# apache/brpc

Hardware: NVIDIA H100
Metric: echo QPS, 1 KB baidu_std (higher is better)
Workload: dtype u8

## Files before the change

brpc_b200/csrc/b2_api.cu:

```cuda
#include <cuda_runtime.h>
#include <dlfcn.h>
#include <stdio.h>
#include <time.h>
#include <stdlib.h>
#include <string.h>
#include <algorithm>
#include <mutex>
#include <string>
#include <unordered_map>
#include <vector>
#include "b2_kernels.cuh"
#include "b2_h2.cuh"

using namespace b2;

static thread_local char g_err[512] = "";
static void set_err(const char* fmt, const char* a = "", const char* b = "") { snprintf(g_err, sizeof g_err, fmt, a, b); }

#define CU(call)                                                                          \
    do {                                                                                  \
        cudaError_t e_ = (call);                                                          \
        if (e_ != cudaSuccess) { set_err("%s: %s", #call, cudaGetErrorString(e_)); return B2_E_CUDA; } \
    } while (0)

// ... 21 lines not shown
    ulonglong2* d_iov = nullptr; b2_iovec* h_iov = nullptr; const void* host_bytes = nullptr;
    uint4* d_refs = nullptr; b2_resp_ref* h_refs = nullptr; int input_mode = B2_INPUT_COPY, resp_mode = B2_RESP_COPY; const uint8_t* pull_bytes = nullptr; uint32_t small_off_refs = 0;
    uint32_t* d_crc_adv = nullptr; unsigned long long* d_counters = nullptr; uint32_t* d_totals = nullptr; DevMethod* d_methods = nullptr;
    size_t meta_tile_off = 0; uint32_t max_tiles = 0; uint32_t n_sms = 132; bool use_tma_pack = true; uint32_t stage_mask = 7;
    StreamPass sp = {}; bool has_streams = false, stream_armed = false, stream_ran = false, stream_valid = false;
    uint32_t st_max = 0, st_open = 0; std::vector<long long> st_keys; std::vector<uint8_t> st_state; std::vector<uint32_t> st_pool, st_pool_free;
    void* d_st_block[10] = {}; void* h_st_mapped[5] = {}; uint32_t* h_st_cnts = nullptr; uint8_t* h_st_out = nullptr; uint8_t* h_st_ctl = nullptr; uint8_t* d_st_ctl = nullptr;
    b2_stream_msg* h_st_msgs = nullptr; b2_stream_event* h_st_events = nullptr; uint8_t* h_st_ctrl = nullptr; uint32_t* h_st_run_ctrl = nullptr;
    cudaEvent_t st_ev[6] = {};
    const uint8_t* st_input = nullptr;
    void* d_sw[4] = {}; size_t sw_have[4] = {}; SwRec* h_sw_recs = nullptr; size_t h_sw_have = 0; uint32_t* h_sw_cnts = nullptr;
    cudaEvent_t sw_ev[8] = {}; bool sw_ran = false;
    b2_run_status* h_run_status = nullptr; b2_msg_desc* h_msgs = nullptr; uint8_t* h_resp = nullptr;
    uint32_t* h_totals = nullptr; uint32_t* h_run_tile_base = nullptr;
    uint32_t n_runs = 0, n_tiles = 0, nbytes = 0, max_run_tiles = 0; uint64_t covered = 0;
    bool uploaded = false, executed = false;
    cudaStream_t stream = nullptr;
    cudaEvent_t ev[kMaxStages + 1];
    const char* stage_names[kMaxStages];
    int n_stages = 0;
    float last_kernel_ms = 0.f; uint32_t last_launches = 0;
    cudaEvent_t ev_first = nullptr, ev_last = nullptr; bool first_pending = true;
    bool profile_stages = false; bool allow_small = true; bool use_fused = true; bool fused_last = false; bool slow_heavy = false;
    bool adaptive_tile = false; bool dense = false; uint32_t avg_frame = 0;
    uint8_t* d_meta = nullptr; uint8_t* h_meta = nullptr;
    uint8_t* d_small = nullptr; uint8_t* h_small = nullptr;
    bool small = false, small_copy_queued = false, use_fused_small = true; uint32_t small_msgs = 0, small_resp = 0, small_off_rs = 0, small_off_msgs = 0, small_off_resp = 0, small_total = 0;
};

static void input_overwritten(b2_ctx* c) { if (c->st_input == c->d_bytes) c->st_input = nullptr; }

static uint32_t g_crc_tab_host[256];
static void crc_table_init() {
    for (uint32_t i = 0; i < 256; i++) {
        uint32_t c = i;
        for (int k = 0; k < 8; k++) c = (c & 1) ? (c >> 1) ^ 0x82f63b78u : (c >> 1);
        g_crc_tab_host[i] = c;
    }
}

extern "C" const char* b2_last_error(void) { return g_err; }
extern "C" const char* b2_version(void) { return "brpc_b200 0.1 (sm_90a)"; }

namespace {
struct BlockPool {
    std::mutex mu;
    static constexpr size_t kSmall = 8192, kSlab = 4u << 20;
// ... 136 lines not shown
    CU(cudaStreamCreateWithFlags(&c->stream, cudaStreamNonBlocking));
    for (int i = 0; i <= kMaxStages; i++) CU(cudaEventCreate(&c->ev[i]));
    CU(cudaEventCreate(&c->ev_first)); CU(cudaEventCreate(&c->ev_last));
    crc_table_init();
    CU(cudaMemcpyToSymbol(c_crc_table, g_crc_tab_host, sizeof g_crc_tab_host));
    {
        std::vector<uint32_t> tab(kCrcHotWords + kCrcTreeWords);
        auto adv = [&](uint32_t x, int bytes) { for (int k = 0; k < bytes; k++) x = g_crc_tab_host[x & 0xff] ^ (x >> 8); return x; };
        for (int k = 0; k < 16; k++) for (uint32_t b = 0; b < 256; b++) tab[k * 256 + b] = adv(g_crc_tab_host[b], k);
        for (int j = 0; j < 4; j++) for (uint32_t b = 0; b < 256; b++) tab[(16 + j) * 256 + b] = adv(b << (8 * j), 512);
        for (int t = 0; t < 5; t++) for (int j = 0; j < 4; j++) for (uint32_t b = 0; b < 256; b++)
            tab[kCrcHotWords + (t * 4 + j) * 256 + b] = adv(b << (8 * j), 16 << t);
        CU(cudaMemcpy(c->d_crc_adv, tab.data(), tab.size() * 4, cudaMemcpyHostToDevice));
    }
    CU(cudaFuncSetAttribute(k_resolve, cudaFuncAttributeMaxDynamicSharedMemorySize, 200 * 1024));
    CU(cudaFuncSetAttribute(k_pack_slow<false>, cudaFuncAttributeMaxDynamicSharedMemorySize, (int)(8 * kSnapRing)));
    CU(cudaFuncSetAttribute(k_pack_tma<kPackGroup>, cudaFuncAttributeMaxDynamicSharedMemorySize, (int)(sizeof(PackWarpSmem) * kPackWarps)));
    CU(cudaFuncSetAttribute(k_pack_tma<kPackGroupSmall>, cudaFuncAttributeMaxDynamicSharedMemorySize, (int)(sizeof(PackWarpSmem) * kPackWarps)));
    if (const char* e = getenv("B2_PACK")) c->use_tma_pack = strcmp(e, "reg") != 0;
    if (const char* e = getenv("B2_SMALL")) c->use_fused_small = strcmp(e, "off") != 0;
    if (const char* e = getenv("B2_FUSED")) c->use_fused = strcmp(e, "off") != 0;
    CU(cudaFuncSetAttribute(k_fused, cudaFuncAttributeMaxDynamicSharedMemorySize, (int)(sizeof(FusedWarpSmem) * (kFusedWarps > kFusedWarpsDense ? kFusedWarps : kFusedWarpsDense))));
    CU(cudaFuncSetAttribute(k_small, cudaFuncAttributeMaxDynamicSharedMemorySize, (int)sizeof(SmallSmem)));
    *out = c;
    return B2_OK;
}

extern "C" int b2_set_server_identity(b2_ctx* c, const char* ip_port) {
    if (!c) return B2_E_INVAL;
    const size_t n = ip_port ? strlen(ip_port) : 0;
    if (n >= sizeof c->cfg.identity) { set_err("identity too long"); return B2_E_INVAL; }
    memset(c->cfg.identity, 0, sizeof c->cfg.identity);
    if (n) memcpy(c->cfg.identity, ip_port, n);
    c->cfg.identity_len = (uint32_t)n;
    return B2_OK;
}

extern "C" int b2_set_modes(b2_ctx* c, int input_mode, int resp_mode) {
    if (!c || (input_mode != B2_INPUT_COPY && input_mode != B2_INPUT_PULL) || (resp_mode != B2_RESP_COPY && resp_mode != B2_RESP_BY_REF && resp_mode != B2_RESP_IOVEC)) { set_err("bad mode"); return B2_E_INVAL; }
    static_assert(sizeof(b2_resp_ref) == sizeof(uint4), "b2_resp_ref is 16 bytes");
    static_assert(sizeof(b2_iovec) == sizeof(ulonglong2) && sizeof(void*) == 8, "b2_iovec is a 16-byte struct iovec");
    if (resp_mode == B2_RESP_IOVEC && !c->d_iov) {
        CU(cudaSetDevice(c->opt.device));
        if (cudaMalloc((void**)&c->d_iov, 32 * (size_t)c->opt.max_msgs) != cudaSuccess || cudaHostAlloc((void**)&c->h_iov, 32 * (size_t)c->opt.max_msgs, cudaHostAllocDefault) != cudaSuccess) {
            cudaFree(c->d_iov); c->d_iov = nullptr; cudaGetLastError(); set_err("allocation of the iovec list failed"); return B2_E_NOMEM;
        }
// ... 52 lines not shown

static BatchPtrs make_ptrs(b2_ctx* c) {
    BatchPtrs B;
    B.bytes = c->d_bytes; B.runs = c->d_runs; B.run_tile_base = c->d_run_tile_base; B.tiles = c->d_tiles;
    B.tile_base = c->d_tile_base; B.tile_scratch = c->d_tile_scratch; B.tile_spec = c->d_tile_spec; B.run_status = c->d_run_status; B.frame_off = c->d_frame_off; B.frame_run = c->d_frame_run; B.frame_row = c->d_frame_row; B.rows = c->d_rows; B.msgs = c->d_msgs;
    B.aux = c->d_aux; B.jobs = c->d_jobs; B.refs = c->d_refs; B.slow_idx = c->d_slow_idx; B.heads = c->d_heads; B.slot = c->d_slot; B.scan_tmp = c->d_scan_tmp; B.resp = c->d_resp; B.unz = c->d_unz; B.snappy_tab = c->d_snappy_tab; B.counters = c->d_counters;
    B.totals = c->d_totals; B.methods = c->d_methods; B.crc_adv = c->d_crc_adv;
    B.n_runs = c->n_runs; B.n_tiles = c->n_tiles; B.max_msgs = c->opt.max_msgs; B.max_resp = c->opt.max_resp_bytes;
    B.runs = reinterpret_cast<const b2_run*>(c->d_meta);
    B.run_tile_base = reinterpret_cast<const uint32_t*>(c->d_meta + (size_t)c->n_runs * sizeof(b2_run));
    B.tile_info = reinterpret_cast<const uint4*>(c->d_meta + c->meta_tile_off);
    if (c->input_mode == B2_INPUT_PULL) B.bytes = c->pull_bytes;
    if (c->small) {
        B.refs = reinterpret_cast<uint4*>(c->d_small + c->small_off_refs);
        B.totals = reinterpret_cast<uint32_t*>(c->d_small);
        B.run_status = reinterpret_cast<b2_run_status*>(c->d_small + c->small_off_rs);
        B.msgs = reinterpret_cast<b2_msg_desc*>(c->d_small + c->small_off_msgs);
        B.resp = c->d_small + c->small_off_resp;
        B.max_msgs = c->small_msgs; B.max_resp = c->small_resp;
    }
    return B;
}

extern "C" int b2_batch_upload(b2_ctx* c, const void* bytes, uint32_t nbytes, const b2_run* runs, uint32_t n_runs) {
    if (!c || (!bytes && nbytes) || (!runs && n_runs)) { set_err("null argument"); return B2_E_INVAL; }
    if ((c->input_mode != B2_INPUT_PULL && nbytes > c->opt.max_batch_bytes) || nbytes >= (1u << 31) || n_runs > c->opt.max_runs) { set_err("batch exceeds ctx capacity"); return B2_E_CAPACITY; }
    uint64_t covered = 0; for (uint32_t r = 0; r < n_runs; r++) covered += runs[r].length;
    if (c->input_mode == B2_INPUT_PULL && covered > c->opt.max_batch_bytes) { set_err("runs exceed ctx capacity"); return B2_E_CAPACITY; }
    c->stream_valid = false;
    c->covered = covered;
    CU(cudaSetDevice(c->opt.device));
    if (c->adaptive_tile) {
        uint32_t t = 8192;
        const uint32_t per_tile = c->input_mode == B2_INPUT_PULL ? 48u : 6u;
        if (c->input_mode == B2_INPUT_PULL && t < 32768) t = 32768;
        while (t < (1u << 20) && t < per_tile * c->avg_frame) t <<= 1;
        c->cfg.tile_bytes = t; c->cfg.tile_shift = 0; while ((1u << c->cfg.tile_shift) < t) c->cfg.tile_shift++;
    }
    const uint32_t shift = c->cfg.tile_shift, tile = c->cfg.tile_bytes;
    c->dense = tile >= 2048 && c->avg_frame && (uint64_t)c->avg_frame * kSpecK < tile;
    c->cfg.spec_k = c->dense ? kSpecKDense : kSpecK;
    uint64_t nt = 0; uint32_t max_rt = 0;
    for (uint32_t r = 0; r < n_runs; r++) {
        if ((runs[r].offset & 15u) || (uint64_t)runs[r].offset + runs[r].length > nbytes) { set_err("run offset must be 16-aligned and inside the batch"); return B2_E_INVAL; }
        c->h_run_tile_base[r] = (uint32_t)nt;
        const uint32_t t = (uint32_t)(((uint64_t)runs[r].length + tile - 1) >> shift);
        nt += t; if (t > max_rt) max_rt = t;
    }
    c->h_run_tile_base[n_runs] = (uint32_t)nt;
    if (nt > c->max_tiles) { set_err("too many tiles"); return B2_E_CAPACITY; }
    c->n_runs = n_runs; c->n_tiles = (uint32_t)nt; c->nbytes = nbytes; c->max_run_tiles = max_rt; c->host_bytes = bytes;
    const size_t tile_off = ((size_t)n_runs * sizeof(b2_run) + 4 * ((size_t)n_runs + 1) + 15) & ~(size_t)15;
    const size_t meta_bytes = tile_off + 16 * (size_t)nt;
    c->meta_tile_off = tile_off;
    if (n_runs) memcpy(c->h_meta, runs, (size_t)n_runs * sizeof(b2_run));
    memcpy(c->h_meta + (size_t)n_runs * sizeof(b2_run), c->h_run_tile_base, 4 * ((size_t)n_runs + 1));
    {
        uint32_t* ti = reinterpret_cast<uint32_t*>(c->h_meta + tile_off);
        for (uint32_t r = 0; r < n_runs; r++) {
            const uint32_t t0 = c->h_run_tile_base[r], t1 = c->h_run_tile_base[r + 1];
            for (uint32_t t = t0; t < t1; t++) { uint32_t* q = ti + 4 * (size_t)t; q[0] = runs[r].offset; q[1] = runs[r].length; q[2] = t - t0; q[3] = r | (runs[r].flags << 24); }
        }
    }
// ... 22 lines not shown

static const char* const kStreamStages[5] = { "stream_route", "stream_alloc", "stream_group", "stream_run", "stream_rst" };
static int launch_stream_pass(b2_ctx* c, const BatchPtrs& B, cudaStream_t s, uint32_t& launches) {
    const StreamPass& S = c->sp;
    const uint32_t msg_bound = c->small ? c->small_msgs : c->opt.max_msgs, sms = c->n_sms;
    auto grid = [&](uint32_t items, uint32_t per_block, uint32_t most) { const uint32_t g = (items + per_block - 1) / per_block; return g < 1 ? 1u : g < most ? g : most; };
    CU(cudaMemsetAsync(S.cnts, 0, 4 * (16 + 2 * (size_t)S.cap), s));
    CU(cudaEventRecord(c->st_ev[0], s));
    k_stream_route<<<grid(msg_bound, 256, sms * 4), 256, 0, s>>>(B, S); CU(cudaEventRecord(c->st_ev[1], s));
    k_stream_alloc<<<grid(c->st_max, 256, sms), 256, 0, s>>>(B, S); CU(cudaEventRecord(c->st_ev[2], s));
    k_stream_group<<<grid(msg_bound, 256, sms * 4), 256, 0, s>>>(B, S); CU(cudaEventRecord(c->st_ev[3], s));
    k_stream_run<<<grid(c->st_max, 4, sms * 8), 128, 0, s>>>(B, S); CU(cudaEventRecord(c->st_ev[4], s));
    k_stream_rst<<<grid(c->n_runs, 4, sms * 4), 128, 0, s>>>(B, S); CU(cudaEventRecord(c->st_ev[5], s));
    CU(cudaMemcpyAsync(c->h_st_cnts, S.cnts, 64, cudaMemcpyDeviceToHost, s));
    launches += 5; c->stream_ran = true; c->st_input = B.bytes;
    return B2_OK;
}

static int launch_pipeline(b2_ctx* c) {
    const BatchPtrs B = make_ptrs(c);
    DevConfig C = c->cfg;
    const bool fused = c->use_fused && !c->slow_heavy && !c->small && c->input_mode == B2_INPUT_COPY && c->resp_mode == B2_RESP_COPY && c->use_tma_pack &&
                       (((uint64_t)c->nbytes + 255) & ~255ull) + 4096 <= c->opt.max_resp_bytes;
    C.fused = fused ? 1u : 0u; C.ovf_base = (c->nbytes + 255u) & ~255u; c->fused_last = fused;
    cudaStream_t s = c->stream;
    int st = 0; uint32_t launches = 0;
    const bool prof = c->profile_stages;
    auto mark = [&](const char* name) { if (prof) { c->stage_names[st] = name; cudaEventRecord(c->ev[st + 1], s); st++; } };
    const uint32_t mask = c->stage_mask;
    if (mask & 1) CU(cudaMemsetAsync(B.totals, 0, 48, s));
    CU(cudaEventRecord(c->ev[0], s));
    c->stream_ran = false;
    if (c->n_runs == 0) { c->n_stages = 0; c->last_launches = 0; return B2_OK; }
    if (c->small && c->use_fused_small && !prof) {
        k_small<<<1, kSmallThreads, sizeof(SmallSmem), s>>>(B, C);
        launches = 1;
        if (c->stream_armed) { int rc = launch_stream_pass(c, B, s, launches); if (rc != B2_OK) return rc; }
        c->stage_names[0] = "fused_small"; cudaEventRecord(c->ev[1], s);
        c->n_stages = 1; c->last_launches = launches;
        CU(cudaGetLastError());
        return B2_OK;
    }
    const uint32_t sms = c->n_sms;
    if (mask & 1) {
    if (c->n_tiles) {
        k_tile_search<<<(c->n_tiles * 32 + 255) / 256, 256, 0, s>>>(B, C); launches++; mark("tile_search");
        if (C.pull) k_tile_walk_pull<<<(uint32_t)(((uint64_t)c->n_tiles * 8 + 127) / 128), 128, 0, s>>>(B, C);
        else k_tile_walk<<<(c->n_tiles + 127) / 128, 128, 0, s>>>(B, C);
        launches++; mark("tile_walk");
    }
    {
        size_t smem = (size_t)c->max_run_tiles * 12;
        if (smem > 200 * 1024) smem = 0;
        k_resolve<<<c->n_runs, 256, smem, s>>>(B, C, smem == 0 ? 1u : 0u); launches++; mark("resolve");
    }
    if (fused) {
        const uint32_t fw = c->avg_frame && !c->dense ? kFusedWarps : kFusedWarpsDense;
        if (c->n_tiles) { k_fused<<<sms, fw * 32, sizeof(FusedWarpSmem) * fw, s>>>(B, C); launches++; mark("fused"); }
    } else {
    if (c->n_tiles) { k_frame_table<<<(uint32_t)(((uint64_t)c->n_tiles * C.spec_k + 255) / 256), 256, 0, s>>>(B, C); launches++; mark("frame_table"); }
    k_decode<<<sms * B2_DECODE_MIN_BLOCKS, kDecodeWarps * 32, 0, s>>>(B, C); launches++; mark("decode");
    k_scan_blocks<<<sms, kScanBlock, 0, s>>>(B); launches++;
    mark("scan");
    }
    }
    if (fused) {
        if (mask & 4) { k_pack_slow<true><<<sms * B2_SLOW_MIN_BLOCKS, 256, 0, s>>>(B, C); launches++; mark("pack_slow"); }
    } else if (c->use_tma_pack) {
        if (mask & 4) {
            if (c->slow_heavy || c->cfg.by_ref) { C.verify_done = 1; k_crc_verify<<<sms * 6, 256, 0, s>>>(B, C); launches++; mark("crc_verify"); }
            k_pack_slow<false><<<sms * B2_SLOW_MIN_BLOCKS, 256, 8 * kSnapRing, s>>>(B, C); launches++; mark("pack_slow");
        }
        if (mask & 2) {
            if ((c->avg_frame && c->avg_frame < 640) || c->cfg.by_ref) k_pack_tma<kPackGroupSmall><<<sms, kPackWarps * 32, sizeof(PackWarpSmem) * kPackWarps, s>>>(B, C);
            else k_pack_tma<kPackGroup><<<sms, kPackWarps * 32, sizeof(PackWarpSmem) * kPackWarps, s>>>(B, C);
            launches++; mark("pack");
        }
    } else { k_pack<<<sms * B2_PACK_MIN_BLOCKS, 256, 0, s>>>(B, C); launches++; mark("pack"); }
    if (c->resp_mode == B2_RESP_IOVEC && !c->small) {
        k_emit_iov<<<sms * 4, 256, 0, s>>>(B, c->d_iov, (unsigned long long)(uintptr_t)c->h_resp, (unsigned long long)(uintptr_t)c->host_bytes);
        launches++; mark("emit_iov");
    }
    if (c->stream_armed) { int rc = launch_stream_pass(c, B, s, launches); if (rc != B2_OK) return rc; }
    if (!prof) { c->stage_names[0] = "pipeline"; cudaEventRecord(c->ev[1], s); st = 1; }
    c->n_stages = st; c->last_launches = launches;
    CU(cudaGetLastError());
    return B2_OK;
}

extern "C" int b2_batch_execute(b2_ctx* c, float* kernel_ms, uint32_t* n_launches) {
    if (!c || !c->uploaded) { set_err("no batch uploaded"); return B2_E_INVAL; }
    CU(cudaSetDevice(c->opt.device));
    if (c->stream_armed) { set_err("a submitted batch of a context with a stream table must be collected first: this entry point replays a batch and does not run the stream pass"); return B2_E_INVAL; }
    c->profile_stages = true;
    int rc = launch_pipeline(c);
    c->profile_stages = false;
    if (rc != B2_OK) return rc;
// ... 1230 lines not shown
```

brpc_b200/csrc/b2_kernels.cuh:

```cuda
#pragma once
#include <cuda_runtime.h>
#include "b2_core.cuh"
#include "b2_inflate.cuh"

namespace b2 {

enum TileKind : uint8_t { kRanOff = 0, kStop = 1, kAmbig = 2 };

struct __align__(16) TileRec {
    uint32_t entry;
    uint32_t exit;
    uint32_t count;
    uint8_t kind;
    int8_t last_proto;
    uint8_t live;
    int8_t pf_in;
};

struct __align__(16) MsgAux {
    uint32_t msg_off;
    uint32_t msg_len;
    uint32_t att_len;
    uint32_t att_off;
    uint32_t cks_off;
// ... 14 lines not shown
constexpr uint32_t kHeadBytes = 96;

enum ErrKind : uint32_t { kErrNone = 0, kErrAttachment, kErrNoService, kErrNoMethod, kErrParseRequest };

struct DevMethod {
    char full_method[200];
    uint32_t full_method_len;
    char service_short[64];  uint32_t service_short_len;
    char service_full[120];  uint32_t service_full_len;
    char request_type[96];   uint32_t request_type_len;
    int32_t handler, echo_attachment, response_checksum_type, response_compress_type;
};
struct DevConfig {
    uint64_t max_body_size;
    uint32_t tile_bytes, tile_shift;
    uint32_t n_methods;
    uint32_t identity_len;
    uint32_t stream_handler;
    uint32_t spec_k;
    uint32_t by_ref;
    uint32_t verify_done;
    uint32_t proto_mask;
    uint32_t fused;
    uint32_t ovf_base;
    uint32_t pull_vecs;
    uint32_t pull;
    char identity[64];
};

struct BatchPtrs {
    const uint8_t* bytes;
    const b2_run* runs;
    const uint32_t* run_tile_base;
    const uint4* tile_info;
    TileRec* tiles;
    uint32_t* tile_base;
    uint32_t* tile_scratch;
    uint32_t* tile_spec;
    b2_run_status* run_status;
    uint32_t* frame_off;
    uint32_t* frame_run;
    uint32_t* frame_row;
    uint4* rows;
    b2_msg_desc* msgs;
    MsgAux* aux;
    PackJob* jobs;
// ... 29 lines not shown
}
struct NoEmit { B2_HD void operator()(uint32_t, const Step&) const {} };
constexpr uint32_t kSpecK = 16;
constexpr uint32_t kSpecKDense = 128;
constexpr uint8_t kKindRewalked = 0x80;
struct EmitSpec {
    uint32_t* out; uint32_t run_off, cap;
    __device__ __forceinline__ void operator()(uint32_t i, const Step& s) const {
        if (i < cap) out[i] = (run_off + s.frame_pos) | ((uint32_t)(s.index != 1) << 31);
    }
};

#if defined(__CUDACC__)

__device__ __forceinline__ uint32_t find_run(const uint32_t* base, uint32_t n_runs, uint32_t tile) {
    uint32_t lo = 0, hi = n_runs;
    while (hi - lo > 1) { const uint32_t mid = (lo + hi) >> 1; if (__ldg(base + mid) <= tile) lo = mid; else hi = mid; }
    return lo;
}
__device__ __forceinline__ bool is_magic(uint32_t w) { return w == kMagicPRPC || w == kMagicSTRM; }
#ifndef B2_SEARCH_FIRST
#define B2_SEARCH_FIRST 2
#endif

__global__ void __launch_bounds__(256, 6) k_tile_search(BatchPtrs B, DevConfig C) {
    const uint32_t warp = (blockIdx.x * blockDim.x + threadIdx.x) >> 5, lane = threadIdx.x & 31;
    if (warp >= B.n_tiles) return;
    const uint4 ti = __ldg(B.tile_info + warp);
    const uint32_t k = ti.z;
    const uint8_t* base = B.bytes + ti.x;
    const uint32_t len = ti.y;
    uint32_t entry = kNone;
    if (k == 0) {
        entry = 0;
    } else {
        const uint32_t t0 = k << C.tile_shift;
        const uint32_t t1 = min(t0 + C.tile_bytes, len);
        for (uint32_t c0 = t0; c0 < t1 && entry == kNone; c0 += (c0 == t0 ? 512u * B2_SEARCH_FIRST : 2048u)) {
            const int nwin = c0 == t0 ? B2_SEARCH_FIRST : 4;
            uint4 v[4]; uint32_t nx[4];
            #pragma unroll
            for (int u = 0; u < 4; u++) {
                const uint32_t p0 = c0 + u * 512 + lane * 16;
                v[u] = make_uint4(0, 0, 0, 0); nx[u] = 0;
                if (u < nwin && p0 < t1) {
                    v[u] = __ldg(reinterpret_cast<const uint4*>(base + p0));
                    nx[u] = __ldg(reinterpret_cast<const uint32_t*>(base + p0 + 16));
                }
// ... 73 lines not shown
            const HdrWords h = pre_pos == pos ? pre : load_hdr_words(run + pos);
            const uint32_t guess = pos + prev_len;
            if (prev_len && guess < tile_end && (uint64_t)guess + 12 <= len) { pre = load_hdr_words(run + guess); pre_pos = guess; }
            else pre_pos = kNone;
            const uint32_t sh = 8u * (pos & 3u);
            const uint32_t h0 = sh ? __funnelshift_r(h.w0, h.w1, sh) : h.w0, h1 = sh ? __funnelshift_r(h.w1, h.w2, sh) : h.w1,
                           h2 = sh ? __funnelshift_r(h.w2, h.w3, sh) : h.w2;
            const int idx = h0 == kMagicPRPC ? 1 : h0 == kMagicSTRM ? 2 : 0;
            const uint32_t body = __byte_perm(h1, 0, 0x0123), meta = __byte_perm(h2, 0, 0x0123);
            if (idx && ((mask >> idx) & 1u) && pf != 12 && (uint64_t)body <= max_body && (uint64_t)(len - pos) >= 12ull + body && meta <= body) {
                s.err = B2_PARSE_OK; s.index = idx; s.pf = idx; s.frame_pos = pos; s.new_pos = pos + 12 + body; s.body = body; s.meta = meta; s.popped = false;
                fast = true;
            }
        }
        if (!fast) s = cut_input_message(run, len, pos, pf, max_body, client, mask);
        if (count == 0 && (s.popped || (s.index != 12 && nshead_claims(run, len, pos, max_body, mask)))) { kind = kAmbig; break; }
        if (s.err != B2_PARSE_OK) { kind = kStop; break; }
        emit(count, s);
        count++; last = s.index; pf = s.index; prev_len = s.new_pos - pos; pos = s.new_pos;
    }
    t.entry = entry; t.exit = pos; t.count = count; t.kind = kind; t.last_proto = (int8_t)last;
}

__global__ void __launch_bounds__(128) k_tile_walk(BatchPtrs B, DevConfig C) {
    const uint32_t t = blockIdx.x * blockDim.x + threadIdx.x;
    if (t >= B.n_tiles) return;
    const uint4 ti = __ldg(B.tile_info + t);
    const uint32_t k = ti.z;
    b2_run run; run.offset = ti.x; run.length = ti.y; run.flags = ti.w >> 24;
    TileRec rec;
    rec.entry = B.tiles[t].entry; rec.exit = 0; rec.count = 0; rec.kind = kStop; rec.last_proto = 0; rec.live = 0; rec.pf_in = -1;
    if (rec.entry != kNone) {
        EmitSpec e; e.out = B.tile_spec + (size_t)t * C.spec_k; e.run_off = run.offset; e.cap = C.spec_k;
        walk_tile_spec(B.bytes + run.offset, run.length, rec.entry, (k + 1) << C.tile_shift, C.max_body_size, (run.flags & B2_RUN_CLIENT) != 0, rec, e, run_mask(C.proto_mask, run.flags));
    }
    B.tiles[t] = rec;
}

__global__ void __launch_bounds__(128) k_tile_walk_pull(BatchPtrs B, DevConfig C) {
    const uint32_t g = blockIdx.x * blockDim.x + threadIdx.x;
    const uint32_t t = g >> 3, sub = threadIdx.x & 7u, lane = threadIdx.x & 31u;
    if (t >= B.n_tiles) return;
    const uint32_t gmask = 0xffu << (lane & 24u), l0 = lane & 24u;
    const uint4 ti = __ldg(B.tile_info + t);
    const uint32_t k = ti.z, len = ti.y;
    const uint8_t* run = B.bytes + ti.x;
    const bool client = ((ti.w >> 24) & B2_RUN_CLIENT) != 0;
// ... 61 lines not shown
        const uint32_t carry = *s_carry;
        if (i < B.n_runs) B.run_status[i].first_msg = carry + wbase + x - v;
        __syncthreads();
        if (threadIdx.x == 0) *s_carry = carry + wtot;
        __syncthreads();
    }
    if (threadIdx.x == 0) { B.totals[0] = *s_carry; if (*s_carry > B.max_msgs) B.totals[2] |= 1u; }
}

constexpr uint32_t kLinkOk = 0x80000000u;
constexpr uint32_t kLinkStop = 0x40000000u;
constexpr uint32_t kLinkEnd = 0x20000000u;
constexpr uint32_t kLinkBroken = 0x10000000u;
constexpr uint32_t kLinkRewalk = 0x08000000u;

__device__ __forceinline__ uint32_t make_link(const TileRec& t, const TileRec* tiles, uint32_t nt, uint32_t shift) {
    if (t.entry == kNone || t.kind == kAmbig) return kLinkRewalk;
    if (t.kind == kStop) return kLinkStop;
    const uint32_t j = t.exit >> shift;
    if (j >= nt) return kLinkEnd;
    return (tiles[j].entry == t.exit ? kLinkOk : kLinkBroken) | j;
}

__global__ void __launch_bounds__(256) k_resolve(BatchPtrs B, DevConfig C, uint32_t use_scratch) {
    extern __shared__ uint32_t sm[];
    const uint32_t r = blockIdx.x;
    const b2_run run = B.runs[r];
    const uint8_t* base = B.bytes + run.offset;
    const uint32_t len = run.length;
    const uint32_t tb = B.run_tile_base[r], nt = B.run_tile_base[r + 1] - tb;
    TileRec* tiles = B.tiles + tb;
    const bool fits = !use_scratch;
    uint32_t* link = fits ? sm : B.tile_scratch + 3ull * tb;
    uint32_t* cp = link + nt;
    uint32_t* live = cp + nt;
    __shared__ uint32_t s_final_pos, s_warp_sum[8], s_warp_pf[8], s_carry_sum, s_carry_pf;
    const uint32_t rmask = run_mask(C.proto_mask, run.flags);
    const bool pf_decides = (run.flags & B2_RUN_CLIENT) && !(rmask & kProtoMaskDump) && (rmask & ~((1u << B2_PROTOCOL_BAIDU_STD) | (1u << B2_PROTOCOL_STREAMING_RPC))) != 0;
    for (uint32_t k = threadIdx.x; k < nt; k += blockDim.x) {
        const TileRec t = tiles[k];
        link[k] = ((k == 0 && t.entry != 0) || pf_decides) ? kLinkRewalk : make_link(t, tiles, nt, C.tile_shift);
        cp[k] = (t.count << 4) | ((uint32_t)t.last_proto & 15u);
        live[k] = 0;
    }
    __shared__ uint32_t s_first_bad;
    if (threadIdx.x == 0) s_first_bad = nt ? nt - 1 : 0;
    __syncthreads();
// ... 621 lines not shown
    for (int d = 1; d < 32; d <<= 1) { const uint32_t y = __shfl_up_sync(0xffffffffu, x, d); if ((threadIdx.x & 31) >= d) x += y; }
    if ((threadIdx.x & 31) == 31) s_warp[threadIdx.x >> 5] = x;
    __syncthreads();
    if (threadIdx.x < 32) {
        uint32_t w = s_warp[threadIdx.x], ws = w;
        #pragma unroll
        for (int d = 1; d < 32; d <<= 1) { const uint32_t y = __shfl_up_sync(0xffffffffu, ws, d); if (threadIdx.x >= d) ws += y; }
        s_warp[threadIdx.x] = ws - w;
        if (threadIdx.x == 31) B.scan_tmp[blk] = ws;
    }
    __syncthreads();
    uint32_t excl = s_warp[threadIdx.x >> 5] + x - sum;
    #pragma unroll
    for (int j = 0; j < kScanItems; j++) { if (base + j < n) B.slot[base + j] = excl; excl += v[j]; }
    __syncthreads();
    }
    __shared__ uint32_t s_ticket, s_carry;
    __threadfence();
    __syncthreads();
    if (threadIdx.x == 0) s_ticket = atomicAdd(B.totals + 5, 1u);
    __syncthreads();
    if (s_ticket == gridDim.x - 1) { __threadfence(); scan_top_body(B, s_warp, &s_carry); }
}
__device__ __forceinline__ void finalize_runs(const BatchPtrs& B, const DevConfig& C) {
    const uint32_t n_msgs = B.totals[0];
    if (C.fused && blockIdx.x == 0 && threadIdx.x == 0) {
        const uint32_t ovf = B.totals[9];
        B.totals[1] = ovf ? C.ovf_base + ovf : C.ovf_base;
    }
    for (uint32_t r = blockIdx.x * blockDim.x + threadIdx.x; r < B.n_runs; r += gridDim.x * blockDim.x) {
        b2_run_status st = B.run_status[r];
        auto off_of = [&](uint32_t i) -> uint32_t {
            if (i >= n_msgs) return B.totals[1];
            return B.slot[i] + B.scan_tmp[i / (kScanBlock * kScanItems)];
        };
        if (C.fused) { st.resp_off = B.runs[r].offset; st.resp_bytes = st.consumed; }
        else {
        st.resp_off = off_of(st.first_msg);
        st.resp_bytes = off_of(st.first_msg + st.n_msgs) - st.resp_off;
        }
        B.run_status[r] = st;
        atomicAdd(B.counters + 0, (unsigned long long)st.consumed);
        atomicAdd(B.counters + 1, (unsigned long long)st.n_msgs);
        atomicAdd(B.counters + 2, (unsigned long long)st.resp_bytes);
        if (st.parse_error != B2_PARSE_ERROR_NOT_ENOUGH_DATA) atomicAdd(B.counters + 4, 1ull);
        if (r == 0) atomicAdd(B.counters + 5, 1ull);
    }
}

__device__ __forceinline__ bool snappy_preamble(const uint8_t* in, uint32_t n, uint32_t& ulen, uint32_t& used) {
    uint32_t v = 0, shift = 0, ip = 0;
    for (;;) {
        if (shift >= 32) return false;
// ... 415 lines not shown
        if (j < 4) b = (uint8_t)(kMagicPRPC >> (8 * j));
        else if (j < 8) b = (uint8_t)(total_body >> (8 * (7 - j)));
        else if (j < 12) b = (uint8_t)(ml >> (8 * (11 - j)));
        else if (j < o_cid) { const uint32_t k = j - 12; b = (k == 0) ? 0x12 : (k == 1) ? 0x02 : (k == 2) ? 0x08 : (k == 4) ? 0x18 : (k == 5) ? (uint8_t)compress_type : 0x00; }
        else if (j == o_cid) b = 0x20;
        else if (j < o_att) b = varint_byte((uint64_t)correlation_id, j - o_cid - 1, cid_n);
        else if (j < o_ct) b = (j == o_att) ? 0x28 : varint_byte(att_len, j - o_att - 1, att_n - 1);
        else if (j < o_ckl) { const uint32_t k = j - o_ct; b = (k == 0) ? 0x50 : (k == 2) ? 0x58 : (k == 3) ? (uint8_t)r_cks_type : (k == 4) ? 0x62 : 0x00; }
        else if (j < o_ckv) b = varint_byte(cks_len, j - o_ckl, ckl_n);
        else if (j < o_pb) b = (r_cks_type == B2_CHECKSUM_TYPE_CRC32C) ? (uint8_t)(crc_be >> (8 * (3 - (j - o_ckv)))) : req_cks[j - o_ckv];
        else if (j == o_pb) b = 0x0a;
        else b = varint_byte(msg_len, j - o_pb - 1, vl);
        out[j] = b;
    }
}

struct CrcTabs;
__device__ __forceinline__ void pack_one(const BatchPtrs& B, const DevConfig& C, uint32_t i, uint32_t lane, const CrcTabs& ct);

__global__ void __launch_bounds__(256, B2_PACK_MIN_BLOCKS) k_pack(BatchPtrs B, DevConfig C) {
    const uint32_t lane = threadIdx.x & 31;
    const uint32_t n_msgs = B.totals[0];
    if (B.totals[2] & 3u) return;
    finalize_runs(B, C);
    __shared__ uint32_t s_hot[kCrcHotWords];
    crc_tabs_to_smem(s_hot, B.crc_adv);
    CrcTabs ct; ct.hot = s_hot; ct.tree = B.crc_adv + kCrcHotWords;
    const uint32_t n_warps = (gridDim.x * blockDim.x) >> 5;
    for (uint32_t i = (blockIdx.x * blockDim.x + threadIdx.x) >> 5; i < n_msgs; i += n_warps) pack_one(B, C, i, lane, ct);
}

__device__ __forceinline__ void pack_one(const BatchPtrs& B, const DevConfig& C, uint32_t i, uint32_t lane, const CrcTabs& ct) {
    const uint32_t bi = i / (kScanBlock * kScanItems);
    const uint32_t slot_off = C.fused ? B.slot[i] : B.slot[i] + B.scan_tmp[bi];
    const b2_msg_desc d = B.msgs[i];
    __syncwarp();
    const bool empty_to_verify = d.status == B2_MSG_RESPONSE && d.error_code == 0 && d.checksum_type == B2_CHECKSUM_TYPE_CRC32C;
    if (d.resp_len == 0 && !empty_to_verify) { if (lane == 0 && d.status != B2_MSG_RESPONSE) B.msgs[i].resp_off = slot_off; return; }
    const MsgAux a = B.aux[i];
    const uint8_t* frame = B.bytes + d.frame_off;
    if (d.status == B2_MSG_REPLAY) {
        uint8_t* out = B.resp + slot_off;
        const uint32_t ml = replay_meta_len(a.svc_len, a.mth_len, d.compress_type, d.correlation_id, a.att_len);
        if (lane == 0) {
            uint8_t* p = out;
            p[0] = 'P'; p[1] = 'R'; p[2] = 'P'; p[3] = 'C'; put_be32(p + 4, ml + a.msg_len); put_be32(p + 8, ml); p += 12;
            const uint32_t rl = 1 + varint_len(a.svc_len) + a.svc_len + 1 + varint_len(a.mth_len) + a.mth_len;
// ... 504 lines not shown
                __syncwarp();
            } else {
                for (uint32_t c0 = lo16; c0 < hi16; c0 += kFusedBuf) {
                    const uint32_t c1 = min(c0 + kFusedBuf, hi16);
                    if (lane == 0) { bulk_wait_read<0>(); mbar_arrive_expect_tx(&S.mbar, c1 - c0); bulk_g2s(S.buf, B.bytes + c0, c1 - c0, &S.mbar); }
                    __syncwarp();
                    mbar_wait(&S.mbar, phase & 1u); phase++;
                    if (o.fast) {
                        const uint32_t p0 = max(o.rs, c0), p1 = min(o.rs + o.prefix, c1);
                        const uint8_t* pf = B.heads + (size_t)i * kHeadBytes;
                        for (uint32_t k = p0; k < p1; k++) S.buf[k - c0] = pf[k - o.rs];
                    }
                    fence_proxy_async();
                    __syncwarp();
                    fused_store(B.resp, S.buf, c0, max(sub_lo, c0), min(sub_hi, c1), lane);
                    if (lane == 0) bulk_commit();
                    __syncwarp();
                }
            }
            sub_lo = sub_hi;
        }
    }
    if (lane == 0) bulk_wait<0>();
}


struct ReqDesc {
    uint32_t kind, flags; int32_t method_idx, timeout_ms; long long correlation_id, log_id;
    int32_t compress_type, checksum_type, frame_type; uint32_t payload_off, payload_len, attachment_off, attachment_len, reserved;
};
__global__ void __launch_bounds__(256) k_pack_requests(const uint8_t* bytes, const ReqDesc* reqs, uint32_t n, const DevMethod* methods, uint32_t n_methods,
                                                       uint8_t* out, const uint32_t* out_offs, uint32_t* out_lens, uint8_t* scratch,
                                                       uint16_t* snappy_tab, const uint32_t* crc_adv) {
    __shared__ uint32_t s_hot[kCrcHotWords];
    crc_tabs_to_smem(s_hot, crc_adv);
    CrcTabs ct; ct.hot = s_hot; ct.tree = crc_adv + kCrcHotWords;
    const uint32_t lane = threadIdx.x & 31, n_warps = (gridDim.x * blockDim.x) >> 5, warp_id = (blockIdx.x * blockDim.x + threadIdx.x) >> 5;
    for (uint32_t i = warp_id; i < n; i += n_warps) {
        const ReqDesc R = reqs[i];
        uint8_t* o = out + out_offs[i];
        const uint8_t* payload = bytes + R.payload_off;
        if (R.kind == 1) {
            uint8_t meta[40]; uint8_t* m = meta;
            *m++ = 0x08; m = put_varint(m, (uint64_t)R.correlation_id);
            if (R.flags & 1u) { *m++ = 0x10; m = put_varint(m, (uint64_t)R.log_id); }
            *m++ = 0x18; m = put_varint(m, (uint64_t)(long long)R.frame_type);
// ... 160 lines not shown
            }
            const uint8_t* uf = bytes + R.user_fields_off;
            for (uint32_t k = 0; k < R.n_user_fields; k++) {
                const uint32_t kl = load_le32(uf), vl = load_le32(uf + 4);
                const uint32_t el = 1 + varint_len(kl) + kl + 1 + varint_len(vl) + vl;
                *p++ = 0x4a; p = put_varint(p, el);
                *p++ = 0x0a; p = put_varint(p, kl); for (uint32_t q = 0; q < kl; q++) *p++ = uf[8 + q];
                *p++ = 0x12; p = put_varint(p, vl); for (uint32_t q = 0; q < vl; q++) *p++ = uf[8 + kl + q];
                uf += 8 + kl + vl;
            }
            *p++ = 0x50; p = put_varint(p, (uint64_t)(long long)R.content_type);
            *p++ = 0x58; p = put_varint(p, (uint64_t)(long long)R.checksum_type);
            *p++ = 0x62; p = put_varint(p, cks_len);
            if (own_cks) p = put_be32(p, crc_be);
            else for (uint32_t k = 0; k < cks_len; k++) *p++ = bytes[R.checksum_value_off + k];
            out_lens[i] = 12 + ml + body_len + att_len;
        }
    }
}

#ifndef B2_SLOW_MIN_BLOCKS
#define B2_SLOW_MIN_BLOCKS 3
#endif
template <bool kLite>
__global__ void __launch_bounds__(256, B2_SLOW_MIN_BLOCKS) k_pack_slow(BatchPtrs B, DevConfig C) {
    const uint32_t lane = threadIdx.x & 31;
    if (B.totals[2] & 3u) return;
    finalize_runs(B, C);
    const uint32_t n_verify = C.verify_done ? 0u : B.totals[7];
    if (B.totals[3] == 0 && n_verify == 0) return;
    __shared__ uint32_t s_hot[kLite ? 1 : kCrcHotWords];
    extern __shared__ __align__(16) uint8_t s_rings[];
    CrcTabs ct; ct.tree = B.crc_adv + kCrcHotWords;
    if (kLite) { ct.hot = B.crc_adv; ct.ring = nullptr; }
    else { crc_tabs_to_smem(s_hot, B.crc_adv); ct.hot = s_hot; ct.ring = s_rings + (threadIdx.x >> 5) * kSnapRing; }
    for (; !C.verify_done;) {
        uint32_t k = 0;
        if (lane == 0) k = atomicAdd(B.totals + 8, 1u);
        k = __shfl_sync(0xffffffffu, k, 0);
        if (k >= n_verify) break;
        const uint32_t i = B.slow_idx[B.max_msgs - 1 - k];
        const uint32_t fo = B.msgs[i].frame_off, meta_size = B.msgs[i].meta_size;
        const uint32_t req_size = B.msgs[i].body_size - meta_size;
        int64_t bwo = (int64_t)req_size - (int64_t)B.msgs[i].attachment_size; if (bwo > (int64_t)req_size) bwo = req_size;
        const uint8_t* frame = B.bytes + fo;
        const uint32_t crc = warp_crc32c_update(0xffffffffu, frame + 12 + meta_size, (uint32_t)bwo, lane, ct) ^ 0xffffffffu;
        const bool good = crc == crc32c_unmask(load_be32(frame + B.aux[i].cks_off));
        if (good) { if (lane == 0) B.jobs[i].fast = 1; }
        else { if (lane == 0) B.jobs[i].fast = 0; __syncwarp(); pack_one(B, C, i, lane, ct); }
    }
    const uint32_t n_slow = B.totals[3];
// ... 695 lines not shown
```

Baseline: 1.017 billion.

## Finalize runs in last fused CTA, bound co-resident kernels, guess frame size early

Moves run finalization into the last-finishing k_fused block via an atomic ticket, so the follow-up slow pack kernel can skip it. Sets shared-memory carveout and tighter launch bounds on several kernels so their blocks fit beside a k_fused CTA, with static asserts on register and smem budgets. Adds a host-side guess of frame size from headers, used before avg_frame is known for tile sizing and kernel selection. Risks extra serialization in the last fused block and register spills from the tighter launch bounds.

```diff
diff --git a/brpc_b200/csrc/b2_api.cu b/brpc_b200/csrc/b2_api.cu
--- a/brpc_b200/csrc/b2_api.cu
+++ b/brpc_b200/csrc/b2_api.cu
@@ -67,7 +67,7 @@
     float last_kernel_ms = 0.f; uint32_t last_launches = 0;
     cudaEvent_t ev_first = nullptr, ev_last = nullptr; bool first_pending = true;
     bool profile_stages = false; bool allow_small = true; bool use_fused = true; bool fused_last = false; bool slow_heavy = false;
-    bool adaptive_tile = false; bool dense = false; uint32_t avg_frame = 0;
+    bool adaptive_tile = false; bool dense = false; uint32_t avg_frame = 0; uint32_t frame_guess = 0;
     uint8_t* d_meta = nullptr; uint8_t* h_meta = nullptr;
     uint8_t* d_small = nullptr; uint8_t* h_small = nullptr;
     bool small = false, small_copy_queued = false, use_fused_small = true; uint32_t small_msgs = 0, small_resp = 0, small_off_rs = 0, small_off_msgs = 0, small_off_resp = 0, small_total = 0;
@@ -250,6 +250,13 @@
     if (const char* e = getenv("B2_FUSED")) c->use_fused = strcmp(e, "off") != 0;
     CU(cudaFuncSetAttribute(k_fused, cudaFuncAttributeMaxDynamicSharedMemorySize, (int)(sizeof(FusedWarpSmem) * (kFusedWarps > kFusedWarpsDense ? kFusedWarps : kFusedWarpsDense))));
     CU(cudaFuncSetAttribute(k_small, cudaFuncAttributeMaxDynamicSharedMemorySize, (int)sizeof(SmallSmem)));
+#ifdef CUDART_VERSION
+    CU(cudaFuncSetAttribute(k_fused, cudaFuncAttributePreferredSharedMemoryCarveout, (int)kFusedCarveoutPct));
+    CU(cudaFuncSetAttribute(k_pack_slow<true>, cudaFuncAttributePreferredSharedMemoryCarveout, (int)kFusedCarveoutPct));
+    CU(cudaFuncSetAttribute(k_tile_search, cudaFuncAttributePreferredSharedMemoryCarveout, (int)kFusedCarveoutPct));
+    CU(cudaFuncSetAttribute(k_tile_walk, cudaFuncAttributePreferredSharedMemoryCarveout, (int)kFusedCarveoutPct));
+    CU(cudaFuncSetAttribute(k_resolve, cudaFuncAttributePreferredSharedMemoryCarveout, (int)kFusedCarveoutPct));
+#endif
     *out = c;
     return B2_OK;
 }
@@ -348,6 +355,19 @@
     return B;
 }
 
+static uint32_t frame_size(const b2_ctx* c) { return c->avg_frame ? c->avg_frame : c->frame_guess; }
+static uint32_t guess_frame_size(const uint8_t* bytes, uint32_t nbytes, const b2_run* runs, uint32_t n_runs) {
+    uint64_t sum = 0; uint32_t n = 0;
+    for (uint32_t r = 0; r < n_runs && n < 64; r++) {
+        if (runs[r].length < 12 || (uint64_t)runs[r].offset + 12 > nbytes) continue;
+        const uint8_t* h = bytes + runs[r].offset;
+        uint32_t magic, be_body; memcpy(&magic, h, 4); memcpy(&be_body, h + 4, 4);
+        if (magic != kMagicPRPC && magic != kMagicSTRM) continue;
+        sum += 12 + (uint64_t)__builtin_bswap32(be_body); n++;
+    }
+    return n ? (uint32_t)(sum / n < (1u << 30) ? sum / n : (1u << 30)) : 0u;
+}
+
 extern "C" int b2_batch_upload(b2_ctx* c, const void* bytes, uint32_t nbytes, const b2_run* runs, uint32_t n_runs) {
     if (!c || (!bytes && nbytes) || (!runs && n_runs)) { set_err("null argument"); return B2_E_INVAL; }
     if ((c->input_mode != B2_INPUT_PULL && nbytes > c->opt.max_batch_bytes) || nbytes >= (1u << 31) || n_runs > c->opt.max_runs) { set_err("batch exceeds ctx capacity"); return B2_E_CAPACITY; }
@@ -356,15 +376,16 @@
     c->stream_valid = false;
     c->covered = covered;
     CU(cudaSetDevice(c->opt.device));
+    if (!c->avg_frame) c->frame_guess = guess_frame_size(static_cast<const uint8_t*>(bytes), nbytes, runs, n_runs);
     if (c->adaptive_tile) {
         uint32_t t = 8192;
         const uint32_t per_tile = c->input_mode == B2_INPUT_PULL ? 48u : 6u;
         if (c->input_mode == B2_INPUT_PULL && t < 32768) t = 32768;
-        while (t < (1u << 20) && t < per_tile * c->avg_frame) t <<= 1;
+        while (t < (1u << 20) && t < per_tile * frame_size(c)) t <<= 1;
         c->cfg.tile_bytes = t; c->cfg.tile_shift = 0; while ((1u << c->cfg.tile_shift) < t) c->cfg.tile_shift++;
     }
     const uint32_t shift = c->cfg.tile_shift, tile = c->cfg.tile_bytes;
-    c->dense = tile >= 2048 && c->avg_frame && (uint64_t)c->avg_frame * kSpecK < tile;
+    c->dense = tile >= 2048 && frame_size(c) && (uint64_t)frame_size(c) * kSpecK < tile;
     c->cfg.spec_k = c->dense ? kSpecKDense : kSpecK;
     uint64_t nt = 0; uint32_t max_rt = 0;
     for (uint32_t r = 0; r < n_runs; r++) {
@@ -433,7 +454,7 @@
     DevConfig C = c->cfg;
     const bool fused = c->use_fused && !c->slow_heavy && !c->small && c->input_mode == B2_INPUT_COPY && c->resp_mode == B2_RESP_COPY && c->use_tma_pack &&
                        (((uint64_t)c->nbytes + 255) & ~255ull) + 4096 <= c->opt.max_resp_bytes;
-    C.fused = fused ? 1u : 0u; C.ovf_base = (c->nbytes + 255u) & ~255u; c->fused_last = fused;
+    C.fused = fused ? 1u : 0u; C.fused_final = 0; C.ovf_base = (c->nbytes + 255u) & ~255u; c->fused_last = fused;
     cudaStream_t s = c->stream;
     int st = 0; uint32_t launches = 0;
     const bool prof = c->profile_stages;
@@ -466,8 +487,8 @@
         k_resolve<<<c->n_runs, 256, smem, s>>>(B, C, smem == 0 ? 1u : 0u); launches++; mark("resolve");
     }
     if (fused) {
-        const uint32_t fw = c->avg_frame && !c->dense ? kFusedWarps : kFusedWarpsDense;
-        if (c->n_tiles) { k_fused<<<sms, fw * 32, sizeof(FusedWarpSmem) * fw, s>>>(B, C); launches++; mark("fused"); }
+        const uint32_t fw = frame_size(c) && !c->dense ? kFusedWarps : kFusedWarpsDense;
+        if (c->n_tiles) { C.fused_final = 1; k_fused<<<sms, fw * 32, sizeof(FusedWarpSmem) * fw, s>>>(B, C); launches++; mark("fused"); }
     } else {
     if (c->n_tiles) { k_frame_table<<<(uint32_t)(((uint64_t)c->n_tiles * C.spec_k + 255) / 256), 256, 0, s>>>(B, C); launches++; mark("frame_table"); }
     k_decode<<<sms * B2_DECODE_MIN_BLOCKS, kDecodeWarps * 32, 0, s>>>(B, C); launches++; mark("decode");
@@ -476,14 +497,14 @@
     }
     }
     if (fused) {
-        if (mask & 4) { k_pack_slow<true><<<sms * B2_SLOW_MIN_BLOCKS, 256, 0, s>>>(B, C); launches++; mark("pack_slow"); }
+        if (mask & 4) { k_pack_slow<true><<<sms * kSlowLiteMinBlocks, kSlowLiteThreads, 0, s>>>(B, C); launches++; mark("pack_slow"); }
     } else if (c->use_tma_pack) {
         if (mask & 4) {
             if (c->slow_heavy || c->cfg.by_ref) { C.verify_done = 1; k_crc_verify<<<sms * 6, 256, 0, s>>>(B, C); launches++; mark("crc_verify"); }
             k_pack_slow<false><<<sms * B2_SLOW_MIN_BLOCKS, 256, 8 * kSnapRing, s>>>(B, C); launches++; mark("pack_slow");
         }
         if (mask & 2) {
-            if ((c->avg_frame && c->avg_frame < 640) || c->cfg.by_ref) k_pack_tma<kPackGroupSmall><<<sms, kPackWarps * 32, sizeof(PackWarpSmem) * kPackWarps, s>>>(B, C);
+            if ((frame_size(c) && frame_size(c) < 640) || c->cfg.by_ref) k_pack_tma<kPackGroupSmall><<<sms, kPackWarps * 32, sizeof(PackWarpSmem) * kPackWarps, s>>>(B, C);
             else k_pack_tma<kPackGroup><<<sms, kPackWarps * 32, sizeof(PackWarpSmem) * kPackWarps, s>>>(B, C);
             launches++; mark("pack");
         }
diff --git a/brpc_b200/csrc/b2_kernels.cuh b/brpc_b200/csrc/b2_kernels.cuh
--- a/brpc_b200/csrc/b2_kernels.cuh
+++ b/brpc_b200/csrc/b2_kernels.cuh
@@ -60,6 +60,7 @@
     uint32_t verify_done;
     uint32_t proto_mask;
     uint32_t fused;
+    uint32_t fused_final;
     uint32_t ovf_base;
     uint32_t pull_vecs;
     uint32_t pull;
@@ -135,8 +136,9 @@
 #ifndef B2_SEARCH_FIRST
 #define B2_SEARCH_FIRST 2
 #endif
-
-__global__ void __launch_bounds__(256, 6) k_tile_search(BatchPtrs B, DevConfig C) {
+constexpr uint32_t kSearchThreads = 256, kSearchMinBlocks = 6, kWalkThreads = 128, kWalkMinBlocks = 12, kResolveThreads = 256, kResolveMinBlocks = 6;
+
+__global__ void __launch_bounds__(kSearchThreads, kSearchMinBlocks) k_tile_search(BatchPtrs B, DevConfig C) {
     const uint32_t warp = (blockIdx.x * blockDim.x + threadIdx.x) >> 5, lane = threadIdx.x & 31;
     if (warp >= B.n_tiles) return;
     const uint4 ti = __ldg(B.tile_info + warp);
@@ -256,7 +258,7 @@
     t.entry = entry; t.exit = pos; t.count = count; t.kind = kind; t.last_proto = (int8_t)last;
 }
 
-__global__ void __launch_bounds__(128) k_tile_walk(BatchPtrs B, DevConfig C) {
+__global__ void __launch_bounds__(kWalkThreads, kWalkMinBlocks) k_tile_walk(BatchPtrs B, DevConfig C) {
     const uint32_t t = blockIdx.x * blockDim.x + threadIdx.x;
     if (t >= B.n_tiles) return;
     const uint4 ti = __ldg(B.tile_info + t);
@@ -364,7 +366,7 @@
     return (tiles[j].entry == t.exit ? kLinkOk : kLinkBroken) | j;
 }
 
-__global__ void __launch_bounds__(256) k_resolve(BatchPtrs B, DevConfig C, uint32_t use_scratch) {
+__global__ void __launch_bounds__(kResolveThreads, kResolveMinBlocks) k_resolve(BatchPtrs B, DevConfig C, uint32_t use_scratch) {
     extern __shared__ uint32_t sm[];
     const uint32_t r = blockIdx.x;
     const b2_run run = B.runs[r];
@@ -1032,13 +1034,13 @@
     __syncthreads();
     if (s_ticket == gridDim.x - 1) { __threadfence(); scan_top_body(B, s_warp, &s_carry); }
 }
-__device__ __forceinline__ void finalize_runs(const BatchPtrs& B, const DevConfig& C) {
+__device__ __forceinline__ void finalize_runs(const BatchPtrs& B, const DevConfig& C, uint32_t tid, uint32_t n_threads) {
     const uint32_t n_msgs = B.totals[0];
-    if (C.fused && blockIdx.x == 0 && threadIdx.x == 0) {
-        const uint32_t ovf = B.totals[9];
+    if (C.fused && tid == 0) {
+        const uint32_t ovf = __ldcg(B.totals + 9);
         B.totals[1] = ovf ? C.ovf_base + ovf : C.ovf_base;
     }
-    for (uint32_t r = blockIdx.x * blockDim.x + threadIdx.x; r < B.n_runs; r += gridDim.x * blockDim.x) {
+    for (uint32_t r = tid; r < B.n_runs; r += n_threads) {
         b2_run_status st = B.run_status[r];
         auto off_of = [&](uint32_t i) -> uint32_t {
             if (i >= n_msgs) return B.totals[1];
@@ -1500,7 +1502,7 @@
     const uint32_t lane = threadIdx.x & 31;
     const uint32_t n_msgs = B.totals[0];
     if (B.totals[2] & 3u) return;
-    finalize_runs(B, C);
+    finalize_runs(B, C, blockIdx.x * blockDim.x + threadIdx.x, gridDim.x * blockDim.x);
     __shared__ uint32_t s_hot[kCrcHotWords];
     crc_tabs_to_smem(s_hot, B.crc_adv);
     CrcTabs ct; ct.hot = s_hot; ct.tree = B.crc_adv + kCrcHotWords;
@@ -2051,6 +2053,15 @@
         }
     }
     if (lane == 0) bulk_wait<0>();
+    __shared__ uint32_t s_ticket;
+    __threadfence();
+    __syncthreads();
+    if (threadIdx.x == 0) s_ticket = atomicAdd(B.totals + 10, 1u);
+    __syncthreads();
+    if (s_ticket == gridDim.x - 1) {
+        __threadfence();
+        if (!(__ldcg(B.totals + 2) & 3u)) finalize_runs(B, C, threadIdx.x, blockDim.x);
+    }
 }
 
 
@@ -2257,11 +2268,21 @@
 #ifndef B2_SLOW_MIN_BLOCKS
 #define B2_SLOW_MIN_BLOCKS 3
 #endif
+constexpr uint32_t kSlowLiteThreads = 128, kSlowLiteMinBlocks = B2_SLOW_MIN_BLOCKS * 256 / kSlowLiteThreads;
+constexpr uint32_t reg_bound(uint32_t threads, uint32_t min_blocks) { return (65536u / (threads * min_blocks)) & ~7u; }
+constexpr uint32_t kFusedFreeRegs = 65536u - B2_FUSED_REGS * kFusedWarps * 32;
+static_assert(reg_bound(kSlowLiteThreads, kSlowLiteMinBlocks) * kSlowLiteThreads <= kFusedFreeRegs, "k_pack_slow<true> must fit beside a k_fused CTA");
+static_assert(reg_bound(kSearchThreads, kSearchMinBlocks) * kSearchThreads <= kFusedFreeRegs, "k_tile_search must fit beside a k_fused CTA");
+static_assert(reg_bound(kWalkThreads, kWalkMinBlocks) * kWalkThreads <= kFusedFreeRegs, "k_tile_walk must fit beside a k_fused CTA");
+static_assert(reg_bound(kResolveThreads, kResolveMinBlocks) * kResolveThreads <= kFusedFreeRegs, "k_resolve must fit beside a k_fused CTA");
+constexpr uint32_t kFusedCarveoutPct = 71, kFusedCarveoutBytes = 164u * 1024;
+constexpr uint32_t kFusedFreeSmem = kFusedCarveoutBytes - 1024 - (uint32_t)(sizeof(FusedWarpSmem) * kFusedWarps + 2 * sizeof(DevMethod) + 128);
+static_assert(kFusedFreeSmem >= 3 * 2048 + 1024 + 128 + 2048 * 12, "a k_fused CTA must leave room for a k_resolve block over a 2048-tile run and a block of each other kernel");
 template <bool kLite>
-__global__ void __launch_bounds__(256, B2_SLOW_MIN_BLOCKS) k_pack_slow(BatchPtrs B, DevConfig C) {
+__global__ void __launch_bounds__(kLite ? kSlowLiteThreads : 256, kLite ? kSlowLiteMinBlocks : B2_SLOW_MIN_BLOCKS) k_pack_slow(BatchPtrs B, DevConfig C) {
     const uint32_t lane = threadIdx.x & 31;
     if (B.totals[2] & 3u) return;
-    finalize_runs(B, C);
+    if (!C.fused_final) finalize_runs(B, C, blockIdx.x * blockDim.x + threadIdx.x, gridDim.x * blockDim.x);
     const uint32_t n_verify = C.verify_done ? 0u : B.totals[7];
     if (B.totals[3] == 0 && n_verify == 0) return;
     __shared__ uint32_t s_hot[kLite ? 1 : kCrcHotWords];
```

Result: faster. 1.032 billion (median of 6 runs) (+1.5%).
